# twesterhout/distributed-matvec

Hardware: AMD Instinct MI355X
Metric: matvecs/sec (higher is better)
Workload: dtype f64; 1 GPU; heisenberg_chain_32: y <- H x, 601080390 basis states, 9927521280 off-diagonal non-zeros, f64 vectors, sigma/x/y resident in HBM; partitions=1, partitioning=single, exchange=none, kernel=direct-pull+staged, x=u(hash(sigma, 42)) - 0.5, exchange_bytes_per_matvec=0

## Files before the change

### distributed-matvec_amd/csrc/host.c

```c
#define _GNU_SOURCE
#include <math.h>
#include <pthread.h>
#include <stdarg.h>
#include <stdio.h>
#include <stdlib.h>
#include <string.h>

#include "../../include/ls_amd.h"
#include "../../include/ls_chpl.h"
#include "../../include/ls_hs.h"
#include "lsk.h"

static __thread char g_last_error[1024] = "";
static ls_amd_error_handler g_handler = NULL;

static int set_error(char const *fmt, ...) {
    va_list ap;
    va_start(ap, fmt);
    vsnprintf(g_last_error, sizeof(g_last_error), fmt, ap);
    va_end(ap);
    return -1;
}
static int dev_error(void) { return set_error("%s", lsk_last_error()); }
int ls_amd_internal_error(char const *fmt, ...) {
// ... 1563 lines not shown
    int has_push_staged;
    int one_rank_full_basis;
    lsk_pairplan pairs;
    void *d_pair_recs, *d_rank_low, *d_pair_binom, *d_states32, *d_pair_rows, *d_pair_sites;
    int global_index;
    int has_hubbard;
    lsk_hubbard hubbard;
    void *d_hub[6];
    int has_chain;
    int chain_cached;
    void *d_chain_cache;
    int chain_wide;
    uint64_t *d_chain_rec;
    void *d_chain_wave;
    int chain_row_bytes;
    double chain_v[2];
    int64_t chain_row0;
    void *d_htab;
    uint32_t *d_slot_of;
    int htab_bits;
    void *d_xs;
    int pull_halo;
    int idx_mode;
    struct ls_amd_gtab *gtab;
    uint64_t *d_vtab;
    int64_t row_g0;
    lsk_pullbuf pbuf;
    int64_t split_rows;
    int64_t split_active;
    int slot_cache, slot_cache_valid;
// ... 450 lines not shown
    int64_t slots = 0, total = 0;
    for (int k = 0; k < 8; ++k) if (lists[k].n > slots) slots = lists[k].n;
    uint64_t *flat = (uint64_t *)calloc((size_t)(8 * slots > 0 ? 8 * slots : 1), sizeof(uint64_t));
    for (int k = 0; k < 8; ++k) {
        for (int64_t q = 0; q < lists[k].n; ++q) { flat[k * slots + q] = lists[k].e[q]; total += (int64_t)(lists[k].e[q] >> 48); }
        free(lists[k].e);
    }
    if (total != n) {
        free(flat);
        return set_error("internal error: tile map covers %lld of %lld rows", (long long)total, (long long)n);
    }
    *out = flat;
    *slots_out = slots;
    return 0;
}
static int build_tilemap(ls_amd_plan *pl, int64_t n, int TILE) {
    uint64_t *flat = NULL;
    int64_t slots = 0;
    char const *e = getenv("LS_AMD_TILE_CHUNK");
    int64_t const chunk = e ? atoll(e) : (TILE >= 512 ? 256 : 0);
    if (tilemap_host(n, TILE, chunk > 0 ? chunk : 0, &flat, &slots) < 0) return -1;
    int const up = upload(&pl->d_tilemap, flat, sizeof(uint64_t) * (size_t)(8 * slots > 0 ? 8 * slots : 1));
    free(flat);
    if (up) return -1;
    pl->tilemap.entries = (uint64_t const *)pl->d_tilemap;
    pl->tilemap.slots_per_xcd = slots;
    return 0;
}
int ls_amd_test_corrupt_plan(ls_amd_plan *pl) {
    if (!pl) return 0;
// ... 14 lines not shown
    return 1;
}
int ls_amd_test_window_find(uint64_t const *reps, int n, uint64_t key) { return lsk_test_window_find(reps, n, key); }
int ls_amd_test_nw_find(uint64_t const *reps, int n, uint64_t key) { return lsk_test_nw_find(reps, n, key); }
int ls_amd_test_chain_near_table(int elem, int ldsp, int16_t *out) { return lsk_test_chain_near_table(elem, ldsp, out); }
uint64_t ls_amd_test_rep_trivial_dihedral(uint64_t a, int L, int inv, int reflect) { return lsk_test_rep_trivial_dihedral(a, L, inv, reflect); }
int ls_amd_bench_k4(int L, int inv, int reflect, int variant, int64_t n, uint64_t const *d_reps, uint64_t *d_out, void *stream) {
    if (lsk_bench_k4(L, inv, reflect, variant, n, d_reps, d_out, stream) != 0) { set_error("%s", lsk_last_error()); return -1; }
    return 0;
}
int64_t ls_amd_test_tilemap(int64_t n, int tile_rows, int64_t chunk, uint64_t **entries) {
    int64_t slots = 0;
    *entries = NULL;
    if (tilemap_host(n, tile_rows, chunk, entries, &slots) < 0) return -1;
    return slots;
}
void ls_amd_test_free(void *p) { free(p); }
int ls_amd_test_gtab_bits(int L, int64_t n) { return lsk_gtab_bits(L, n, (int64_t)1 << 40); }
int ls_amd_test_gtab_build(int L, int bbits, int64_t n, uint64_t const *reps, uint32_t const *payload, uint64_t **entries) {
    lsk_gtab t;
    t.entries = NULL; t.L = L; t.bbits = bbits; t.tbits = L - bbits;
    *entries = (uint64_t *)malloc(sizeof(uint64_t) * ((size_t)2 << bbits));
    if (lsk_test_gtab_build_host(t, *entries, n, reps, payload) != 0) { free(*entries); *entries = NULL; return -1; }
    return 0;
}
int64_t ls_amd_test_gtab_find(int L, int bbits, uint64_t const *entries, uint64_t key) {
    lsk_gtab t;
    t.entries = NULL; t.L = L; t.bbits = bbits; t.tbits = L - bbits;
    return lsk_test_gtab_find(t, entries, key);
}
// ... 38 lines not shown
    for (int w = 0; w < 4096; ++w) {
        int const k = __builtin_popcount(w);
        rank_in[w] = (uint16_t)(pos[k] - class_off[k]);
        U[pos[k]++] = (uint16_t)w;
    }
    for (int w = 0; w < 4096; ++w) Rg[w] = low_site >= 0 ? rank_in[w ^ (1 << low_site)] : 0;
}
int ls_amd_test_chain_wave_tables(int low_site, uint16_t *U, uint16_t *Rg, int *class_off) {
    if (low_site >= 12) return set_error("ls_amd_test_chain_wave_tables: the low site lies below bit 12");
    chain_wave_tables(low_site, U, Rg, class_off);
    return 0;
}
static int setup_chain_headers(ls_amd_plan *pl, lsk_index index, int64_t n, uint64_t const *d_reps, int nc, uint64_t xmask, void *stream) {
    int const L = NBITS(pl->op->basis);
    char const *e = getenv("LS_AMD_CHAIN_RECORDS");
    int headed = !(e && atoi(e) != 0) && L >= 13 && L <= 32 && pl->dbs.proj == LSK_PROJ_NONE && pl->chain_row0 == 0 &&
                 pl->family == FAMILY_DIRECT_PULL && pl->dbs.hamming_weight >= 0 && nc <= 1;
    int lo = -1, hi = -1;
    if (headed && nc == 1) {
        lo = __builtin_ctzll(xmask);
        hi = 63 - __builtin_clzll(xmask);
        if (lo >= 12 || hi < 12) { headed = 0; lo = hi = -1; }
    }
    int const words = lsk_chain_words();
    int64_t const n_hdr = (n + 63) / 64;
    uint16_t U[4096], Rg[4096];
    int class_off[14];
    uint32_t *tab = (uint32_t *)malloc(sizeof(uint32_t) * (size_t)words);
    if (!tab) return set_error("out of memory");
    chain_wave_tables(headed ? lo : -1, U, Rg, class_off);
    for (int t = 0; t < words; ++t) tab[t] = (uint32_t)U[t] | ((uint32_t)Rg[U[t]] << 16) | (lo >= 0 ? (((uint32_t)U[t] >> lo) & 1u) << 31 : 0u);
    size_t const tab_bytes = sizeof(uint32_t) * (size_t)words, hdr_bytes = 8 * (size_t)n_hdr;
    void *q;
    if (lsk_malloc(&q, tab_bytes + hdr_bytes + 8) != 0) { free(tab); return 1; }
    unsigned long long plain = 0;
    unsigned long long *d_plain = (unsigned long long *)((char *)q + tab_bytes + hdr_bytes);
    int const rc = lsk_h2d(q, tab, tab_bytes) || lsk_h2d(d_plain, &plain, 8) ||
                   lsk_chain_headers(pl->dbs, index, n, d_reps, headed, hi, (char *)q + tab_bytes, d_plain, stream) || lsk_sync(stream) ||
                   lsk_d2h(&plain, d_plain, 8);
    free(tab);
    if (rc) { lsk_free(q); return dev_error(); }
    pl->d_chain_wave = q;
    int const rec = pl->cplx ? 4 + 4 * nc : 8;
    pl->chain_row_bytes = headed ? (int)((8 * (uint64_t)n_hdr + 64 * (uint64_t)rec * (uint64_t)plain + (uint64_t)n - 1) / (uint64_t)n) : rec;
    return 0;
}
static int setup_chain(ls_amd_plan *pl, lsk_index index, int64_t n, uint64_t const *d_reps, void *stream) {
    struct ls_amd_operator_ext const *ext = OEXT(pl->op);
    int nc = ext->n_groups - ext->runs.n_run_groups;
    int const Ls = NBITS(pl->op->basis);
    int const inv = pl->dbs.proj == LSK_PROJ_INVERSION;
    uint64_t const top = 1ULL << (Ls - 1);
    uint64_t cx[3];
    double cv[3];
    int k = 0;
    if (inv)
        for (int q = 0; q < pl->dop.runs.n_runs; ++q)
            if (pl->dop.runs.lo0[q] + pl->dop.runs.cnt[q] - 1 == Ls - 2) {
                cx[k] = 3ULL << (Ls - 2);
// ... 49 lines not shown
        pl->d_chain_rec = (uint64_t *)q;
        DEV(lsk_chain_pack(n, d_reps, pl->chain_cached ? pl->d_chain_cache : NULL, (uint64_t *)q, stream));
        DEV(lsk_sync(stream));
        if (pl->chain_cached <= 1 && pl->d_chain_cache) { lsk_free(pl->d_chain_cache); pl->d_chain_cache = NULL; }
    }
    if (NBITS(pl->op->basis) <= 32 && !pl->chain_wide && n > 0) {
        int const rc = setup_chain_headers(pl, index, n, d_reps, pl->chain_cached, pl->chain_cached > 0 ? cx[0] : 0, stream);
        if (rc < 0) return -1;
        if (rc > 0) {
            if (pl->d_chain_rec) { lsk_free(pl->d_chain_rec); pl->d_chain_rec = NULL; }
            if (pl->d_chain_cache) { lsk_free(pl->d_chain_cache); pl->d_chain_cache = NULL; }
            if (pl->d_tilemap) { lsk_free(pl->d_tilemap); pl->d_tilemap = NULL; memset(&pl->tilemap, 0, sizeof(pl->tilemap)); }
            pl->chain_cached = 0;
            return 0;
        }
    }
    pl->has_chain = 1;
    return 0;
}

static int pair_cmp(void const *pa, void const *pb) {
    lsk_pair const *a = (lsk_pair const *)pa, *b = (lsk_pair const *)pb;
    int const ca = a->j < 11 ? 0 : (a->i < 11 ? 1 : 2), cb = b->j < 11 ? 0 : (b->i < 11 ? 1 : 2);
    if (ca != cb) return ca - cb;
    if (a->i != b->i) return (int)a->i - (int)b->i;
    return (int)a->j - (int)b->j;
}
static int setup_pairs(ls_amd_plan *pl, int64_t n, uint64_t const *d_reps, void *stream) {
    ls_hs_operator const *op = pl->op;
    struct ls_amd_operator_ext const *ext = OEXT(op);
// ... 815 lines not shown
            if (ps->d_soff) lsk_free(ps->d_soff);
            if (ps->scatter_gt) ls_amd_internal_gtab_release(ps->scatter_gt);
            free(ps->h_soff);
            free(ps->ttab_first);
            free(ps->send_counts); free(ps->h_beta_off); free(ps->h_val_off);
        }
        free(pl->parts);
    }
    if (pl->d_gtable) lsk_free(pl->d_gtable);
    if (pl->d_row_gidx) lsk_free(pl->d_row_gidx);
    if (pl->d_norms_global) lsk_free(pl->d_norms_global);
    if (pl->d_tilemap) lsk_free(pl->d_tilemap);
    if (pl->d_chain_cache) lsk_free(pl->d_chain_cache);
    if (pl->d_chain_rec) lsk_free(pl->d_chain_rec);
    if (pl->d_chain_wave) lsk_free(pl->d_chain_wave);
    if (pl->d_pair_recs) lsk_free(pl->d_pair_recs);
    for (int k = 0; k < 6; ++k) if (pl->d_hub[k]) lsk_free(pl->d_hub[k]);
    if (pl->d_pair_rows) lsk_free(pl->d_pair_rows);
    if (pl->d_pair_sites) lsk_free(pl->d_pair_sites);
    if (pl->d_rank_low) lsk_free(pl->d_rank_low);
    if (pl->d_pair_binom) lsk_free(pl->d_pair_binom);
    if (pl->d_states32) lsk_free(pl->d_states32);
    if (pl->d_htab) lsk_free(pl->d_htab);
    if (pl->d_slot_of) lsk_free(pl->d_slot_of);
    if (pl->d_xs) lsk_free(pl->d_xs);
    if (pl->gtab) ls_amd_internal_gtab_release(pl->gtab);
    split_free(pl);
    block_free(pl);
    if (pl->d_send) lsk_free(pl->d_send);
    if (pl->d_cursors) lsk_free(pl->d_cursors);
// ... 269 lines not shown
    default: return pl->streams ? "tile+streams" : (pl->has_push_staged ? "tile(one rank: push+staged)" : "tile");
    }
}
int ls_amd_plan_packet_bytes(ls_amd_plan const *pl) { return pl->key_bytes + (pl->cplx ? 16 : 8); }
int ls_amd_plan_row_bytes(ls_amd_plan const *pl) {
    if (pl->has_hubbard) return 0;
    if (pl->has_pairs) return pl->pairs.wide ? 8 : 4;
    if (pl->has_chain) {
        if (pl->d_chain_wave) return pl->chain_row_bytes;
        int const narrow = NBITS(pl->op->basis) <= 32 && !pl->chain_wide;
        return (narrow ? 4 : 8) + pl->chain_cached * (pl->chain_wide ? 8 : 4);
    }
    if (pl->family == FAMILY_TILE_PULL || pl->family == FAMILY_REPL_TILE) return 16;
    return 8;
}
int64_t ls_amd_plan_nnz(ls_amd_plan const *pl) { return pl->nnz; }
int ls_amd_plan_send_counts(ls_amd_plan const *pl, int round, int64_t *counts) {
    if (pl->family != FAMILY_TILE) { for (int d = 0; d < pl->P; ++d) counts[d] = 0; return 0; }
    part_state const *ps = &pl->parts[0];
    if (round < 0 || round >= ps->rounds) return set_error("round out of range");
    memcpy(counts, ps->send_counts + (size_t)round * pl->P, sizeof(int64_t) * pl->P);
    return 0;
}

static int prescaled_x(ls_amd_plan *pl, int64_t n, uint64_t const *d_reps, void const *d_x, double const *d_norms,
                       void const **out, void *stream) {
    if (!pl->d_htab) {
        int bits = 4;
        while (((int64_t)1 << bits) < 2 * n) ++bits;
        if (bits > 32) return set_error("hash index: more than 2^31 representatives per table are not supported");
// ... 231 lines not shown
            int const st = stage_begin(pl, ST_DIAG, stream);
            DEV(lsk_memset_async(d_y[0], 0, (size_t)pl->parts[0].count * (pl->cplx ? 16 : 8), stream));
            stage_end(pl, st, stream);
        }
    } else if (pl->family != FAMILY_DIRECT_PULL) {
        int const st = stage_begin(pl, ST_DIAG, stream);
        for (int p = 0; p < pl->n_local; ++p)
            DEV(lsk_diag(pl->dop, pl->cplx, pl->parts[p].count, pl->parts[p].d_reps, d_x[p], d_y[p], stream));
        stage_end(pl, st, stream);
    }
    if (pl->dop.n_groups == 0 && pl->family != FAMILY_DIRECT_PULL) return 0;
    if (pl->family != FAMILY_TILE) {
        part_state *ps = &pl->parts[0];
        int const st = stage_begin(pl, ST_ROWS, stream);
        int slot = timing_begin(pl, stream);
        if (pl->has_chain)
            DEV(lsk_chain(pl->dop, pl->dbs, ps->index, pl->cplx, pl->chain_wide, pl->d_chain_rec != NULL, pl->tilemap, ps->count,
                          pl->d_chain_rec ? pl->d_chain_rec : ps->d_reps, 0, ps->count, d_x[0], d_y[0], pl->chain_cached,
                          pl->d_chain_cache, pl->chain_v[0], pl->chain_v[1], pl->d_chain_wave, stream));
        else if (pl->has_pairs)
            DEV(lsk_pairs(pl->pairs, pl->dbs.hamming_weight, pl->cplx, pl->tilemap, ps->count, d_x[0], d_y[0], stream));
        else if (pl->has_hubbard)
            DEV(lsk_hubbard_apply(pl->hubbard, pl->dop, pl->cplx, pl->tilemap, d_x[0], d_y[0], stream));
        else if (pl->has_push_staged)
            DEV(lsk_push_staged(pl->dop, pl->dbs, ps->index, pl->cplx, pl->tilemap, ps->count, ps->d_reps, d_x[0], d_y[0], pl->d_err, stream));
        else
            DEV(lsk_direct(pl->dop, pl->dbs, ps->index, pl->cplx, pl->family == FAMILY_DIRECT_PULL ? (OEXT(pl->op)->is_hermitian ? 1 : 2) : 0, pl->tilemap, ps->d_reps,
                           d_x[0], d_y[0], pl->d_err, stream));
        timing_end(pl, slot, stream);
        stage_end(pl, st, stream);
        return 0;
    }
    int const P = pl->P;
    if (pl->streams) {
        uint64_t const *d_binom;
// ... 2959 lines not shown
```

### distributed-matvec_amd/csrc/k_rows.hip

```cpp
#include <hip/hip_runtime.h>
#include "lsk_dev.hpp"

template <bool CPLX>
__global__ __launch_bounds__(kBlock) void k_diag(lsk_runs runs, int n_diag, lsk_term const *__restrict__ diag,
                                                 int64_t n, uint64_t const *__restrict__ reps,
                                                 double const *__restrict__ x, double *__restrict__ y) {
    for (int64_t i = (int64_t)blockIdx.x * kBlock + threadIdx.x; i < n; i += (int64_t)gridDim.x * kBlock) {
        uint64_t a = reps[i];
        double dr, di;
        diag_coeff<uint64_t, false>(runs, n_diag, diag, a, dr, di);
        if (CPLX) {
            double xr = x[2 * i], xi = x[2 * i + 1];
            y[2 * i] = dr * xr - di * xi;
            y[2 * i + 1] = dr * xi + di * xr;
        } else {
            y[i] = dr * x[i];
        }
    }
}

extern "C" int lsk_diag(lsk_operator op, int cplx, int64_t n, uint64_t const *reps, void const *x, void *y,
                        void *stream) {
    if (n == 0 || op.n_diag == 0) return 0;
    dim3 g(grid_for(n)), b(kBlock);
// ... 531 lines not shown
}

constexpr int kChainHalo = 512;
constexpr int kChainLdsPairs = 12;
constexpr int kChainFar = 12;
constexpr uint32_t kChainWords = 4096;

__device__ __forceinline__ double cx_load_nt(double const *p) { return __builtin_nontemporal_load(p); }
__device__ __forceinline__ double2 cx_load_nt(double2 const *p) {
    typedef double d2v __attribute__((ext_vector_type(2)));
    const d2v v = __builtin_nontemporal_load(reinterpret_cast<d2v const *>(p));
    return make_double2(v.x, v.y);
}
constexpr int kChainFarC = 6;

template <typename W, typename R, bool CPLX, int TILE, bool REC>
__global__ __launch_bounds__(kBlock, (CPLX || sizeof(R) == 8 ? 5 : (sizeof(W) == 8 ? 6 : 7))) void k_chain_t(lsk_runs runs, int n_diag, lsk_term const *__restrict__ diag,
                                                    int hamming_weight, uint4 const *__restrict__ g_img, int img16, int kc,
                                                    int near_off,
                                                    uint64_t const *__restrict__ tilemap, int64_t slots_per_xcd, int64_t n,
                                                    uint64_t const *__restrict__ reps, void const *__restrict__ x_v,
                                                    void *__restrict__ y_v, int n_cached,
                                                    R const *__restrict__ cache, double cv0, double cv1, int64_t row0,
                                                    int64_t n_x, uint32_t const *__restrict__ wave_plan) {
    typedef typename ChainX<CPLX>::type X;
    typedef WordTraits<W> WT;
    constexpr int NB = ChainTraits<W, R>::NB;
    constexpr int HALO = CPLX ? 256 : kChainHalo;
    constexpr int LDSP = CPLX ? 11 : kChainLdsPairs;
    constexpr int WINDOW = TILE + 2 * HALO + 2;
    constexpr int FAR = CPLX ? kChainFarC : kChainFar;
    constexpr R kNone = ~(R)0;
    constexpr int hb = kChainLdsPairs;
    X const *__restrict__ x = (X const *)x_v;
    X *__restrict__ y = (X *)y_v;
    const bool extra_stream = kAblate && (n_cached & 0x100);
    const int nt_from = !kAblate ? 99 : ((n_cached & 0x200) ? 20 : ((n_cached & 0x400) ? 0 : 99));
    if (kAblate) n_cached &= 0xff;
    uint64_t ex_next = 0;
    extern __shared__ uint4 s_img[];
    R const *const s_binom = reinterpret_cast<R const *>(s_img);
    uint2 const *const s_near = reinterpret_cast<uint2 const *>(reinterpret_cast<char const *>(s_img) + near_off);
    __shared__ X s_x[WINDOW + 1];
    for (int k = threadIdx.x; k < img16; k += kBlock) s_img[k] = g_img[k];
    (void)NB;
    if (threadIdx.x == 0) s_x[WINDOW] = cx_zero<X>();
    const int xcd = blockIdx.x & 7;
    const int64_t blocks_per_xcd = gridDim.x >> 3;
    const int lane = threadIdx.x & 63;
    tilemap += (int64_t)xcd * slots_per_xcd;
    uint32_t const *__restrict__ reps32 = reinterpret_cast<uint32_t const *>(reps);
    constexpr bool HDR = REC || (CPLX && sizeof(W) == 4 && sizeof(R) == 4);
    constexpr int NSUB = TILE / kBlock;
    for (int64_t t = blockIdx.x >> 3; t < slots_per_xcd; t += blocks_per_xcd) {
        const uint64_t slot = tilemap[t];
        const int cnt = (int)(slot >> 48);
        if (cnt == 0) continue;
        const int64_t i0 = (int64_t)(slot & 0xffffffffffffULL);
        const int64_t w0 = (row0 + i0 - HALO) & ~(int64_t)1;
        W a_next = 0;
        R t0_next = kNone, t1_next = kNone;
        auto load_row = [&](int64_t row, W &a_out, R &t0_out, R &t1_out) {
            if (REC) {
                const uint64_t rec = __builtin_nontemporal_load(reps + row);
                a_out = (W)(uint32_t)rec;
                t0_out = (R)(uint32_t)(rec >> 32);
            } else {
                if (sizeof(W) == 4) a_out = (W)__builtin_nontemporal_load(reps32 + 2 * row);
                else a_out = (W)__builtin_nontemporal_load(reps + row);
                if (n_cached > 0) t0_out = __builtin_nontemporal_load(cache + row);
            }
            if (n_cached > 1) t1_out = __builtin_nontemporal_load(cache + (size_t)n + (size_t)row);
            if (kAblate && extra_stream) ex_next = __builtin_nontemporal_load(reps + (row < (n >> 1) ? row + (n >> 1) : row - (n >> 1)));
        };
        const int wave0 = (int)(threadIdx.x & ~63u);
        uint32_t hq = ~0u;
        if (HDR) {
            const uint32_t hw = 2 * (uint32_t)(i0 >> 6) + 2 * ((threadIdx.x >> 6) + (uint32_t)(lane % NSUB) * (kBlock / 64)) + (lane / NSUB) % 2;
            if (((int64_t)(hw >> 1) << 6) < n) hq = wave_plan[kChainWords + hw];
        }
        auto fetch_row = [&](int s, int64_t row) {
            if (HDR) {
                const uint32_t ti = (uint32_t)__builtin_amdgcn_readlane((int)hq, s) & (kChainWords - 1u);
                if (ti != kChainWords - 1u) { a_next = (W)wave_plan[ti + lane]; return; }
            }
            load_row(row, a_next, t0_next, t1_next);
        };
        if (wave0 < cnt) {
            const int64_t rr = i0 + ((int)threadIdx.x < cnt ? (int)threadIdx.x : cnt - 1);
            fetch_row(0, rr);
        }
        __syncthreads();
        if (CPLX) {
            for (int j = threadIdx.x; j < WINDOW; j += kBlock) {
                const int64_t row = w0 + j;
                s_x[j] = (row >= 0 && row < n_x) ? x[row] : cx_zero<X>();
            }
        } else {
            double const *xd = (double const *)x_v;
            double *sd = (double *)s_x;
            for (int j = 2 * threadIdx.x; j < WINDOW; j += 2 * kBlock) {
                const int64_t row = w0 + j;
                double2 v;
                if (row >= 0 && row + 1 < n_x) v = *reinterpret_cast<double2 const *>(xd + row);
                else { v.x = (row >= 0 && row < n_x) ? xd[row] : 0.0; v.y = (row + 1 >= 0 && row + 1 < n_x) ? xd[row + 1] : 0.0; }
                sd[j] = v.x;
                sd[j + 1] = v.y;
            }
        }
        __syncthreads();
        const int own0 = (int)(row0 + i0 - w0);
        X y_pending = cx_zero<X>();
        int r_pending = -1;
#pragma unroll 1
        for (int sub = 0; sub < TILE / kBlock; ++sub) {
            const int r = sub * kBlock + threadIdx.x;
            if (r_pending >= 0) cx_store_nt(y + i0 + r_pending, y_pending);
            r_pending = -1;
            W a = a_next;
            R t0 = t0_next;
            const R t1 = t1_next;
            const uint64_t ex = ex_next;
            if (sub + 1 < TILE / kBlock && (sub + 1) * kBlock + wave0 < cnt) {
                const int64_t in = i0 + (r + kBlock < cnt ? r + kBlock : cnt - 1);
                fetch_row(sub + 1, in);
            }
            if (sub * kBlock + wave0 >= cnt) continue;
            const bool ghost = r >= cnt;
            const int64_t i = i0 + (ghost ? cnt - 1 : r);
            const R ig = (R)(row0 + i);
            W a0;
            int ubit;
            const uint32_t h0 = HDR ? (uint32_t)__builtin_amdgcn_readlane((int)hq, sub) : ~0u;
            if (HDR && (h0 & (kChainWords - 1u)) != kChainWords - 1u) {
                const uint32_t word = (uint32_t)a;
                a0 = (W)(h0 & ~(kChainWords - 1u));
                a = a0 | (W)(word & (kChainWords - 1u));
                ubit = 0;
                const uint32_t h1 = (uint32_t)__builtin_amdgcn_readlane((int)hq, NSUB + sub);
                t0 = (int32_t)(word ^ h1) < 0 ? (R)((h1 & 0x7fffffffu) + ((word >> 16) & 0x7fffu)) : kNone;
            } else {
                a0 = readfirstlane_t<W>(a);
                const W adiff = a0 ^ readlane_t<W>(a, 63);
                ubit = adiff == 0 ? 0 : (int)(8 * sizeof(W)) - (sizeof(W) == 4 ? __clz((int)(uint32_t)adiff) : __clzll((long long)(uint64_t)adiff));
            }
            const int jr = own0 + (int)(i - i0);
            const X xr = s_x[jr];
            X g0 = n_cached > 0 ? xr : cx_zero<X>(), g1 = n_cached > 1 ? xr : cx_zero<X>();
            if (t0 != kNone) g0 = x[t0];
            if (n_cached > 1 && t1 != kNone) g1 = x[t1];
            double dr, di;
            diag_coeff<W, true>(runs, n_diag, diag, a, dr, di);
            X acc = cx_scale(dr, xr);
            const W tdiff = a ^ (a >> 1);
            const R ig0 = readfirstlane_t<R>(ig);
            const uint32_t dl = (uint32_t)(ig - ig0);
            for (int q = 0; q < runs.n_runs; ++q) {
                const int lo0 = runs.lo0[q];
                int lo_end = lo0 + runs.cnt[q];
                const double vr = runs.v_re[q];
                int k = WT::popc(a & (W)(((uint64_t)1 << lo0) - 1));
                int lo = lo0;
                const int e1 = lo_end < LDSP ? lo_end : LDSP;
                const int near_end = lo0 > e1 ? lo0 : e1;
                int split = hb == 0 ? lo_end : (hb < near_end ? near_end : (hb > lo_end ? lo_end : hb));
                if (hb != 0 && split < ubit) split = ubit < lo_end ? ubit : lo_end;
                const bool uni = split < lo_end;
                unsigned long long m = 0;
                R off = 0;
                X xv[FAR];
#pragma unroll
                for (int u = 0; u < FAR; ++u) xv[u] = cx_zero<X>();
                if (uni) {
                    const int p = split + lane;
                    const bool in_run = p < lo_end;
                    const int ps = in_run ? p : 0;
                    const W hi = a0 >> ps;
                    const bool bit = hi & 1;
                    const bool act = in_run && (((hi >> 1) & 1) != (W)bit);
                    const int kk = hamming_weight - WT::popc(hi);
                    const R d = s_binom[ps * kc + (kk < 0 ? 0 : kk)];
                    off = bit ? d : (R)(0 - d);
                    m = __builtin_amdgcn_ballot_w64(act);
#pragma unroll
                    for (int u = 0; u < FAR; ++u) {
                        if (m) {
                            const int l = __builtin_ctzll(m);
                            m &= m - 1;
                            X const *const src = x + (size_t)(R)(ig0 + readlane_t<R>(off, l)) + dl;
                            if (kAblate && split + l >= nt_from) xv[u] = cx_load_nt(src); else xv[u] = *src;
                        }
                    }
                    lo_end = split;
                }
// ... 23 lines not shown
                        for (int u = 0; u < NBATCH; ++u)
                            if (p0 + u < LDSP) cx_fma(vr, nv[u], acc);
                    }
                    lo = LDSP;
                    k = __popc(al & ((1u << LDSP) - 1u));
                }
#pragma unroll 4
                for (; lo < e1; ++lo) {
                    const bool bit = (a >> lo) & 1;
                    const bool act = (tdiff >> lo) & 1;
                    const int d = (int)s_binom[lo * kc + k];
                    k += bit ? 1 : 0;
                    const int j = bit ? jr + d : jr - d;
                    cx_fma(vr, s_x[act ? j : WINDOW], acc);
                }
#pragma unroll
                for (int u = 0; u < FAR; ++u) cx_fma(vr, xv[u], acc);
                while (m) {
                    X xw[4];
#pragma unroll
                    for (int u = 0; u < 4; ++u) {
                        xw[u] = cx_zero<X>();
                        if (m) {
                            const int l = __builtin_ctzll(m);
                            m &= m - 1;
                            xw[u] = (x + (size_t)(R)(ig0 + readlane_t<R>(off, l)))[dl];
                        }
                    }
#pragma unroll
                    for (int u = 0; u < 4; ++u) cx_fma(vr, xw[u], acc);
                }
#pragma unroll 4
                for (; lo < lo_end; ++lo) {
                    const bool bit = (a >> lo) & 1;
                    const bool act = (tdiff >> lo) & 1;
                    const R d = s_binom[lo * kc + k];
                    k += bit ? 1 : 0;
                    R idx = bit ? (R)(ig + d) : (R)(ig - d);
                    idx = act ? idx : ig;
                    cx_fma(act ? vr : 0.0, x[idx], acc);
                }
            }
            cx_fma(t0 != kNone ? cv0 : 0.0, g0, acc);
            cx_fma(t1 != kNone ? cv1 : 0.0, g1, acc);
            if (kAblate && extra_stream && ex == 0x0123456789abcdefULL) cx_fma(1.0, xr, acc);
            y_pending = acc;
            r_pending = ghost ? -1 : r;
        }
        if (r_pending >= 0) cx_store_nt(y + i0 + r_pending, y_pending);
    }
}

template <typename W, typename R>
__global__ __launch_bounds__(kBlock) void k_chain_cache(int64_t n, uint64_t const *__restrict__ reps, uint64_t xmask, uint64_t inv_mask,
                                                        int hamming_weight, uint64_t const *__restrict__ g_binom,
                                                        R *__restrict__ out, int *__restrict__ flag) {
    constexpr int NB = ChainTraits<W, R>::NB;
    __shared__ R s_binom[NB * LSK_BINOM_K];
    for (int k = threadIdx.x; k < NB * LSK_BINOM_K; k += blockDim.x) s_binom[k] = (R)g_binom[k];
    __syncthreads();
    for (int64_t i = (int64_t)blockIdx.x * kBlock + threadIdx.x; i < n; i += (int64_t)gridDim.x * kBlock) {
        const W a = (W)reps[i];
        R t = ~(R)0;
        if (WordTraits<W>::popc(a & (W)xmask) == 1) {
            W beta = a ^ (W)xmask;
// ... 176 lines not shown
    if (n == 0 || tm.slots_per_xcd == 0) return 0;
    const bool narrow = bs.number_sites <= 32 && !wide_ranks;
    if ((wave_plan != nullptr) != narrow) { snprintf(g_err, sizeof(g_err), "lsk_chain: 32-bit states and ranks come with wave headers, the other plans without"); return -1; }
#define LSK_CHAIN_ARGS op, bs, ix, tm, n, reps, row0, n_x, x, y, n_cached, cache, cv0, cv1, wave_plan, stream
    if (fused_records) {
        if (!narrow || cplx) { snprintf(g_err, sizeof(g_err), "lsk_chain: fused records need 32-bit states and ranks and f64 vectors"); return -1; }
        return launch_chain<uint32_t, uint32_t, false, 1024, true>(LSK_CHAIN_ARGS);
    }
    if (narrow) {
        if (!cplx) { snprintf(g_err, sizeof(g_err), "lsk_chain: 32-bit states and ranks with f64 vectors run on fused records (lsk_chain_pack)"); return -1; }
        return launch_chain<uint32_t, uint32_t, true, 512, false>(LSK_CHAIN_ARGS);
    }
    if (!wide_ranks) return cplx ? launch_chain<uint64_t, uint32_t, true, 512, false>(LSK_CHAIN_ARGS) : launch_chain<uint64_t, uint32_t, false, 1024, false>(LSK_CHAIN_ARGS);
    return cplx ? launch_chain<uint64_t, uint64_t, true, 512, false>(LSK_CHAIN_ARGS) : launch_chain<uint64_t, uint64_t, false, 1024, false>(LSK_CHAIN_ARGS);
#undef LSK_CHAIN_ARGS
}

constexpr int kPairLowBits = 11;
constexpr int kPairHalo = 512;
constexpr int kPairFar = 8;
enum { PAIR_NEAR = 0, PAIR_STRADDLE = 1, PAIR_HIGH = 2 };

template <typename SW, bool CPLX, int TILE>
__global__ __launch_bounds__(kBlock, (CPLX ? 4 : 6)) void k_pairs_t(lsk_pairplan pp, int hamming_weight, uint64_t const *__restrict__ tilemap,
                                                              int64_t slots_per_xcd, int64_t n, void const *__restrict__ x_v,
                                                              void *__restrict__ y_v) {
    typedef typename ChainX<CPLX>::type X;
    constexpr int HALO = kPairHalo;
    constexpr int WINDOW = TILE + 2 * HALO + 2;
    constexpr int LOWMASK = (1 << kPairLowBits) - 1;
// ... 452 lines not shown
```

### distributed-matvec_amd/csrc/lsk.h

```cpp
#ifndef LSK_H
#define LSK_H

#include <stddef.h>
#include <stdint.h>

#ifdef __cplusplus
extern "C" {
#endif

#define LSK_BENES_STAGES 11
#define LSK_BINOM_K 34
#define LSK_MAX_PARTS 256

typedef struct lsk_term {
    double v_re, v_im;
    uint64_t m, r, s;
} lsk_term;

enum { LSK_GROUP_GENERIC = 0, LSK_GROUP_EXCHANGE = 1,
       LSK_GROUP_HOP_LO = 2, LSK_GROUP_HOP_HI = 3 };

typedef struct lsk_group {
    uint64_t x;
    double v_re, v_im;
// ... 150 lines not shown
int lsk_event_destroy(void *ev);
int lsk_event_record(void *ev, void *stream);
int lsk_event_elapsed_ms(void *start, void *stop, float *ms);

int lsk_fill_random(int64_t n, uint64_t const *states, uint64_t seed, int cplx, void *out, void *stream);

int lsk_diag(lsk_operator op, int cplx, int64_t n, uint64_t const *reps, void const *x, void *y,
             void *stream);
int lsk_direct_validate(lsk_operator op, lsk_basis bs, lsk_index ix, int64_t n, uint64_t const *reps, int *d_err, void *stream);
int lsk_direct(lsk_operator op, lsk_basis bs, lsk_index ix, int cplx, int pull, lsk_tilemap tm,
               uint64_t const *reps, void const *x, void *y, int *d_err, void *stream);
int lsk_chain_tile_rows(int cplx);
int lsk_chain(lsk_operator op, lsk_basis bs, lsk_index ix, int cplx, int wide_ranks, int fused_records, lsk_tilemap tm,
              int64_t n, uint64_t const *reps, int64_t row0, int64_t n_x, void const *x, void *y, int n_cached,
              void const *cache, double cv0, double cv1, void const *wave_plan, void *stream);
#define LSK_MAX_PAIRS 128
#define LSK_PAIR_KC 20
typedef struct lsk_pair {
    uint8_t i, j, pad[6];
    double v;
    double vz;
} lsk_pair;
typedef struct lsk_pair_row {
    uint64_t between;
    double v, vz;
    int i, j;
} lsk_pair_row;
#define LSK_PAIR_SITE_MAX_DEGREE 8
#define LSK_PAIR_SITE_MAX_CLASSES 64
typedef struct lsk_pairplan {
// ... 375 lines not shown
```

### include/ls_amd.h

```cpp
#ifndef LS_AMD_H
#define LS_AMD_H

#include "ls_hs.h"

#ifdef __cplusplus
extern "C" {
#endif

typedef enum { LS_AMD_F64 = 0, LS_AMD_C128 = 1 } ls_amd_dtype;

typedef enum {
    LS_AMD_MODE_AUTO = 0,
    LS_AMD_MODE_PUSH = 1,
    LS_AMD_MODE_PULL = 2
} ls_amd_mode;

typedef struct ls_amd_plan ls_amd_plan;

char const *ls_amd_last_error(void);
typedef void (*ls_amd_error_handler)(char const *message);
void ls_amd_set_error_handler(ls_amd_error_handler handler);

int ls_amd_device_count(void);
int ls_amd_set_device(int device);
// ... 245 lines not shown
int ls_amd_expect_matrix_elements(ls_amd_expect *plan, ls_amd_dtype dtype, int Ka, void const *d_bra, int64_t bra_row, int64_t bra_col,
                                  int Kb, void const *d_ket, int64_t ket_row, int64_t ket_col, double *h_out, void *stream);
char const *ls_amd_expect_matrix_kernel_name(ls_amd_expect const *plan, int Ka, int Kb);
int64_t ls_amd_test_expect_average(ls_hs_basis const *basis, ls_hs_operator const *op, int64_t cap, double *v, uint64_t *m, uint64_t *r,
                                   uint64_t *x, uint64_t *s);

int ls_amd_basis_group_order(ls_hs_basis const *basis);
int ls_amd_basis_fermion_signs(ls_hs_basis const *basis);
int ls_amd_test_fermion_sign(ls_hs_basis const *basis, int element, uint64_t state, int table);
int ls_amd_basis_spin_flip(ls_hs_basis const *basis);
int ls_amd_test_group_element_kind(ls_hs_basis const *basis, int element);
uint64_t ls_amd_basis_apply_group_element(ls_hs_basis const *basis, int element, uint64_t state);
int ls_amd_basis_group_character(ls_hs_basis const *basis, int element, double *re, double *im);

int64_t ls_amd_test_tilemap(int64_t n, int tile_rows, int64_t chunk, uint64_t **entries);
void ls_amd_test_free(void *p);
int ls_amd_test_window_find(uint64_t const *reps, int n, uint64_t key);
int ls_amd_test_nw_find(uint64_t const *reps, int n, uint64_t key);
int ls_amd_test_chain_near_table(int elem, int ldsp, int16_t *out);
int ls_amd_test_chain_wave_tables(int low_site, uint16_t *U, uint16_t *Rg, int *class_off);
uint64_t ls_amd_test_rep_trivial_dihedral(uint64_t a, int L, int inv, int reflect);
int ls_amd_bench_k4(int L, int inv, int reflect, int variant, int64_t n, uint64_t const *d_reps, uint64_t *d_out, void *stream);
int ls_amd_test_translation_cosets(ls_hs_basis const *basis, int *n_cosets);
uint64_t ls_amd_test_rep_by_cosets(ls_hs_basis const *basis, uint64_t state);
int ls_amd_test_d4_mask(ls_hs_basis const *basis);
int ls_amd_test_gtab_bits(int L, int64_t n);
int ls_amd_test_gtab_build(int L, int bbits, int64_t n, uint64_t const *reps, uint32_t const *payload, uint64_t **entries);
int64_t ls_amd_test_gtab_find(int L, int bbits, uint64_t const *entries, uint64_t key);
int ls_amd_test_primme_comminfo_offset(void);
int ls_amd_test_primme_sumtype_offset(void);
// ... 8 lines not shown
```

Baseline: 142.2 matvecs/s.

## Pair chain tiles across the top-bond offset so far hops stay in LDS

For the Heisenberg chain, rows in a middle index range whose top-bond (site L-2) hop lands a fixed distance d away are processed in paired tiles. Each tile loads two x windows into LDS, one at i0 and one at i0+d, so the top-bond partner and most bit-LDSP hops are read from shared memory instead of through gathered global loads. A separate tile map covers the remaining rows, and a second kernel launch with its own header array handles the paired rows. The cost is more setup, a larger LDS window per block, and an extra launch. Correctness now depends on the binomial ordering of the basis.

```diff
diff --git a/distributed-matvec_amd/csrc/host.c b/distributed-matvec_amd/csrc/host.c
--- a/distributed-matvec_amd/csrc/host.c
+++ b/distributed-matvec_amd/csrc/host.c
@@ -1601,6 +1601,12 @@
     uint64_t *d_chain_rec;
     void *d_chain_wave;
     int chain_row_bytes;
+    int chain_headed;
+    int chain_headers_apply;
+    int chain_paired;
+    void *d_tilemap_pair, *d_chain_hdr_b;
+    lsk_tilemap tilemap_pair;
+    int64_t chain_pair_d, chain_pair_a0, chain_pair_rows;
     double chain_v[2];
     int64_t chain_row0;
     void *d_htab;
@@ -2081,6 +2087,64 @@
     *slots_out = slots;
     return 0;
 }
+static int chain_pair_range(int L, int k, int64_t *a0, int64_t *a1, int64_t *d) {
+    if (L < 14 || L > 32 || k < 1 || k > L - 1) return 0;
+    uint64_t C[33][33];
+    memset(C, 0, sizeof(C));
+    for (int n = 0; n <= 32; ++n) { C[n][0] = 1; for (int j = 1; j <= n; ++j) C[n][j] = C[n - 1][j - 1] + (j <= n - 1 ? C[n - 1][j] : 0); }
+    int64_t const r01 = (int64_t)C[L - 2][k], r10 = (int64_t)C[L - 1][k];
+    *d = r10 - r01;
+    *a0 = (r01 + 511) & ~(int64_t)511;
+    *a1 = r10 & ~(int64_t)511;
+    return *a1 > *a0;
+}
+#define CHAIN_TILE_PLAIN 0x8000
+static int tilemap_deal(tile_list const *all, int64_t chunk, uint64_t **out, int64_t *slots_out) {
+    int64_t const tiles = all->n;
+    int64_t per[8] = {0, 0, 0, 0, 0, 0, 0, 0}, slots = 0;
+    if (chunk > 0) for (int64_t q = 0; q < tiles; ++q) ++per[(q / chunk) % 8];
+    else for (int k = 0; k < 8; ++k) per[k] = tiles * (k + 1) / 8 - tiles * k / 8;
+    for (int k = 0; k < 8; ++k) if (per[k] > slots) slots = per[k];
+    uint64_t *flat = (uint64_t *)calloc((size_t)(8 * slots > 0 ? 8 * slots : 1), sizeof(uint64_t));
+    if (!flat) return set_error("out of memory");
+    int64_t fill[8] = {0, 0, 0, 0, 0, 0, 0, 0};
+    int k0 = 0;
+    for (int64_t q = 0; q < tiles; ++q) {
+        int k;
+        if (chunk > 0) k = (int)((q / chunk) % 8);
+        else { while (q >= tiles * (k0 + 1) / 8) ++k0; k = k0; }
+        flat[k * slots + fill[k]++] = all->e[q];
+    }
+    *out = flat;
+    *slots_out = slots;
+    return 0;
+}
+static int tilemap_paired_host(int64_t n, int TILE, int64_t chunk, int64_t a0, int64_t a1, int64_t d, uint64_t **rest, int64_t *rest_slots,
+                               uint64_t **pairs, int64_t *pair_slots) {
+    tile_list all[2];
+    memset(all, 0, sizeof(all));
+    int64_t const piece[3][2] = {{0, a0}, {a1, a0 + d}, {a1 + d, n}};
+    int64_t total = 0;
+    for (int p = 0; p < 3; ++p)
+        for (int64_t pos = piece[p][0]; pos < piece[p][1];) {
+            int64_t end = (pos / TILE + 1) * TILE;
+            if (pos & 63) end = (pos | 63) + 1;
+            if (end > piece[p][1]) end = piece[p][1];
+            int const plain = (pos & 63) != 0 || ((end & 63) != 0 && end != n);
+            tile_push(&all[0], pos, (end - pos) | (plain ? CHAIN_TILE_PLAIN : 0));
+            total += end - pos;
+            pos = end;
+        }
+    for (int64_t i0 = a0; i0 < a1; i0 += 512) { tile_push(&all[1], i0, 1024); total += 1024; }
+    int rc = total == n ? 0 : set_error("internal error: paired tile maps cover %lld of %lld rows", (long long)total, (long long)n);
+    *rest = *pairs = NULL;
+    if (!rc) rc = tilemap_deal(&all[0], chunk, rest, rest_slots);
+    if (!rc) rc = tilemap_deal(&all[1], chunk, pairs, pair_slots);
+    if (rc) { free(*rest); free(*pairs); *rest = *pairs = NULL; }
+    free(all[0].e);
+    free(all[1].e);
+    return rc;
+}
 static int build_tilemap(ls_amd_plan *pl, int64_t n, int TILE) {
     uint64_t *flat = NULL;
     int64_t slots = 0;
@@ -2125,6 +2189,15 @@
     *entries = NULL;
     if (tilemap_host(n, tile_rows, chunk, entries, &slots) < 0) return -1;
     return slots;
+}
+int ls_amd_test_tilemap_paired(int L, int weight, int tile_rows, int64_t chunk, uint64_t **rest, uint64_t **pairs, int64_t *out) {
+    int64_t a0, a1, d, n = 1;
+    *rest = *pairs = NULL;
+    if (!chain_pair_range(L, weight, &a0, &a1, &d)) return 0;
+    for (int j = 1; j <= weight; ++j) n = n * (L - weight + j) / j;
+    if (tilemap_paired_host(n, tile_rows, chunk, a0, a1, d, rest, &out[4], pairs, &out[5]) != 0) return -1;
+    out[0] = n; out[1] = a0; out[2] = a1; out[3] = d;
+    return 1;
 }
 void ls_amd_test_free(void *p) { free(p); }
 int ls_amd_test_gtab_bits(int L, int64_t n) { return lsk_gtab_bits(L, n, (int64_t)1 << 40); }
@@ -2193,7 +2266,7 @@
 static int setup_chain_headers(ls_amd_plan *pl, lsk_index index, int64_t n, uint64_t const *d_reps, int nc, uint64_t xmask, void *stream) {
     int const L = NBITS(pl->op->basis);
     char const *e = getenv("LS_AMD_CHAIN_RECORDS");
-    int headed = !(e && atoi(e) != 0) && L >= 13 && L <= 32 && pl->dbs.proj == LSK_PROJ_NONE && pl->chain_row0 == 0 &&
+    int headed = L >= 13 && L <= 32 && pl->dbs.proj == LSK_PROJ_NONE && pl->chain_row0 == 0 &&
                  pl->family == FAMILY_DIRECT_PULL && pl->dbs.hamming_weight >= 0 && nc <= 1;
     int lo = -1, hi = -1;
     if (headed && nc == 1) {
@@ -2201,6 +2274,8 @@
         hi = 63 - __builtin_clzll(xmask);
         if (lo >= 12 || hi < 12) { headed = 0; lo = hi = -1; }
     }
+    pl->chain_headers_apply = headed;
+    if (e && atoi(e) != 0) { headed = 0; lo = hi = -1; }
     int const words = lsk_chain_words();
     int64_t const n_hdr = (n + 63) / 64;
     uint16_t U[4096], Rg[4096];
@@ -2220,8 +2295,59 @@
     free(tab);
     if (rc) { lsk_free(q); return dev_error(); }
     pl->d_chain_wave = q;
+    pl->chain_headed = headed;
     int const rec = pl->cplx ? 4 + 4 * nc : 8;
     pl->chain_row_bytes = headed ? (int)((8 * (uint64_t)n_hdr + 64 * (uint64_t)rec * (uint64_t)plain + (uint64_t)n - 1) / (uint64_t)n) : rec;
+    return 0;
+}
+static int setup_chain_pairs(ls_amd_plan *pl, lsk_index index, int64_t n, uint64_t const *d_reps, int hi, void *stream) {
+    char const *e = getenv("LS_AMD_CHAIN_PAIRED");
+    int const L = NBITS(pl->op->basis);
+    if ((e && atoi(e) == 0) || !pl->chain_headers_apply || pl->cplx || !pl->d_chain_rec || pl->chain_cached > 1 || pl->chain_row0 != 0 ||
+        pl->n_local != 1 || pl->family != FAMILY_DIRECT_PULL)
+        return 0;
+    int top = 0;
+    for (int q = 0; q < pl->dop.runs.n_runs; ++q)
+        if (pl->dop.runs.lo0[q] <= L - 2 && L - 2 < pl->dop.runs.lo0[q] + pl->dop.runs.cnt[q]) top = 1;
+    int64_t a0, a1, d;
+    if (!top || !chain_pair_range(L, pl->dbs.hamming_weight, &a0, &a1, &d) || a1 + d > n) return 0;
+    uint64_t *rest = NULL, *pairs = NULL;
+    int64_t rest_slots = 0, pair_slots = 0;
+    char const *ce = getenv("LS_AMD_TILE_CHUNK");
+    int64_t const chunk = ce ? atoll(ce) : 256;
+    if (tilemap_paired_host(n, lsk_chain_tile_rows(0), chunk > 0 ? chunk : 0, a0, a1, d, &rest, &rest_slots, &pairs, &pair_slots) != 0) return -1;
+    void *d_rest = NULL, *d_pairs = NULL, *d_hdr = NULL;
+    int64_t const n_b = a1 - a0;
+    unsigned long long plain = 0;
+    int rc = lsk_malloc(&d_rest, sizeof(uint64_t) * (size_t)(8 * rest_slots > 0 ? 8 * rest_slots : 1)) ||
+             lsk_malloc(&d_pairs, sizeof(uint64_t) * (size_t)(8 * pair_slots)) || lsk_malloc(&d_hdr, 8 * (size_t)(n_b / 64) + 8);
+    if (!rc) {
+        unsigned long long *d_plain = (unsigned long long *)((char *)d_hdr + 8 * (size_t)(n_b / 64));
+        rc = lsk_h2d(d_rest, rest, sizeof(uint64_t) * (size_t)(8 * rest_slots)) || lsk_h2d(d_pairs, pairs, sizeof(uint64_t) * (size_t)(8 * pair_slots)) ||
+             lsk_h2d(d_plain, &plain, 8) || lsk_chain_headers(pl->dbs, index, n_b, d_reps + a0 + d, pl->chain_headed, hi, d_hdr, d_plain, stream) ||
+             lsk_sync(stream);
+        if (rc) { free(rest); free(pairs); lsk_free(d_rest); lsk_free(d_pairs); lsk_free(d_hdr); return dev_error(); }
+    }
+    free(rest);
+    free(pairs);
+    if (rc) {
+        if (d_rest) lsk_free(d_rest);
+        if (d_pairs) lsk_free(d_pairs);
+        if (d_hdr) lsk_free(d_hdr);
+        return 0;
+    }
+    lsk_free(pl->d_tilemap);
+    pl->d_tilemap = d_rest;
+    pl->tilemap.entries = (uint64_t const *)d_rest;
+    pl->tilemap.slots_per_xcd = rest_slots;
+    pl->d_tilemap_pair = d_pairs;
+    pl->tilemap_pair.entries = (uint64_t const *)d_pairs;
+    pl->tilemap_pair.slots_per_xcd = pair_slots;
+    pl->d_chain_hdr_b = d_hdr;
+    pl->chain_pair_d = d;
+    pl->chain_pair_a0 = a0;
+    pl->chain_pair_rows = 2 * (a1 - a0);
+    pl->chain_paired = 1;
     return 0;
 }
 static int setup_chain(ls_amd_plan *pl, lsk_index index, int64_t n, uint64_t const *d_reps, void *stream) {
@@ -2301,6 +2427,7 @@
             pl->chain_cached = 0;
             return 0;
         }
+        if (setup_chain_pairs(pl, index, n, d_reps, pl->chain_cached > 0 ? 63 - __builtin_clzll(cx[0]) : -1, stream) != 0) return -1;
     }
     pl->has_chain = 1;
     return 0;
@@ -3146,6 +3273,8 @@
     if (pl->d_chain_cache) lsk_free(pl->d_chain_cache);
     if (pl->d_chain_rec) lsk_free(pl->d_chain_rec);
     if (pl->d_chain_wave) lsk_free(pl->d_chain_wave);
+    if (pl->d_tilemap_pair) lsk_free(pl->d_tilemap_pair);
+    if (pl->d_chain_hdr_b) lsk_free(pl->d_chain_hdr_b);
     if (pl->d_pair_recs) lsk_free(pl->d_pair_recs);
     for (int k = 0; k < 6; ++k) if (pl->d_hub[k]) lsk_free(pl->d_hub[k]);
     if (pl->d_pair_rows) lsk_free(pl->d_pair_rows);
@@ -3445,6 +3574,9 @@
     if (pl->family == FAMILY_TILE_PULL || pl->family == FAMILY_REPL_TILE) return 16;
     return 8;
 }
+int64_t ls_amd_plan_chain_paired_rows(ls_amd_plan const *pl) {
+    return pl->has_chain && pl->chain_paired ? pl->chain_pair_rows : 0;
+}
 int64_t ls_amd_plan_nnz(ls_amd_plan const *pl) { return pl->nnz; }
 int ls_amd_plan_send_counts(ls_amd_plan const *pl, int round, int64_t *counts) {
     if (pl->family != FAMILY_TILE) { for (int d = 0; d < pl->P; ++d) counts[d] = 0; return 0; }
@@ -3706,11 +3838,14 @@
         part_state *ps = &pl->parts[0];
         int const st = stage_begin(pl, ST_ROWS, stream);
         int slot = timing_begin(pl, stream);
-        if (pl->has_chain)
+        if (pl->has_chain) {
             DEV(lsk_chain(pl->dop, pl->dbs, ps->index, pl->cplx, pl->chain_wide, pl->d_chain_rec != NULL, pl->tilemap, ps->count,
                           pl->d_chain_rec ? pl->d_chain_rec : ps->d_reps, 0, ps->count, d_x[0], d_y[0], pl->chain_cached,
                           pl->d_chain_cache, pl->chain_v[0], pl->chain_v[1], pl->d_chain_wave, stream));
-        else if (pl->has_pairs)
+            if (pl->chain_paired)
+                DEV(lsk_chain_paired(pl->dop, pl->dbs, pl->tilemap_pair, ps->count, pl->d_chain_rec, d_x[0], d_y[0], pl->chain_cached, pl->chain_v[0],
+                                     pl->d_chain_wave, pl->chain_pair_d, pl->chain_pair_a0, pl->d_chain_hdr_b, NBITS(pl->op->basis) - 2, stream));
+        } else if (pl->has_pairs)
             DEV(lsk_pairs(pl->pairs, pl->dbs.hamming_weight, pl->cplx, pl->tilemap, ps->count, d_x[0], d_y[0], stream));
         else if (pl->has_hubbard)
             DEV(lsk_hubbard_apply(pl->hubbard, pl->dop, pl->cplx, pl->tilemap, d_x[0], d_y[0], stream));
diff --git a/distributed-matvec_amd/csrc/k_rows.hip b/distributed-matvec_amd/csrc/k_rows.hip
--- a/distributed-matvec_amd/csrc/k_rows.hip
+++ b/distributed-matvec_amd/csrc/k_rows.hip
@@ -569,21 +569,25 @@
 }
 constexpr int kChainFarC = 6;
 
-template <typename W, typename R, bool CPLX, int TILE, bool REC>
-__global__ __launch_bounds__(kBlock, (CPLX || sizeof(R) == 8 ? 5 : (sizeof(W) == 8 ? 6 : 7))) void k_chain_t(lsk_runs runs, int n_diag, lsk_term const *__restrict__ diag,
+struct chain_pair_args { int64_t d, a0; uint32_t const *hdr_b; int bond; };
+template <typename W, typename R, bool CPLX, int TILE, bool REC, bool PAIR>
+__device__ __forceinline__ void chain_rows(lsk_runs const &runs, int n_diag, lsk_term const *__restrict__ diag,
                                                     int hamming_weight, uint4 const *__restrict__ g_img, int img16, int kc,
                                                     int near_off,
                                                     uint64_t const *__restrict__ tilemap, int64_t slots_per_xcd, int64_t n,
                                                     uint64_t const *__restrict__ reps, void const *__restrict__ x_v,
                                                     void *__restrict__ y_v, int n_cached,
                                                     R const *__restrict__ cache, double cv0, double cv1, int64_t row0,
-                                                    int64_t n_x, uint32_t const *__restrict__ wave_plan) {
+                                                    int64_t n_x, uint32_t const *__restrict__ wave_plan, chain_pair_args const &pr) {
     typedef typename ChainX<CPLX>::type X;
     typedef WordTraits<W> WT;
     constexpr int NB = ChainTraits<W, R>::NB;
-    constexpr int HALO = CPLX ? 256 : kChainHalo;
-    constexpr int LDSP = CPLX ? 11 : kChainLdsPairs;
-    constexpr int WINDOW = TILE + 2 * HALO + 2;
+    constexpr int HALO = (CPLX || PAIR) ? 256 : kChainHalo;
+    constexpr int LDSP = (CPLX || PAIR) ? 11 : kChainLdsPairs;
+    constexpr int SEG = TILE / 2;
+    constexpr int WSEG = SEG + 2 * HALO + 2;
+    constexpr int WINDOW = PAIR ? 2 * WSEG : TILE + 2 * HALO + 2;
+    static_assert(!PAIR || (REC && !CPLX && SEG % kBlock == 0 && SEG % 64 == 0), "paired tiles: f64 on fused records");
     constexpr int FAR = CPLX ? kChainFarC : kChainFar;
     constexpr R kNone = ~(R)0;
     constexpr int hb = kChainLdsPairs;
@@ -609,10 +613,13 @@
     constexpr int NSUB = TILE / kBlock;
     for (int64_t t = blockIdx.x >> 3; t < slots_per_xcd; t += blocks_per_xcd) {
         const uint64_t slot = tilemap[t];
-        const int cnt = (int)(slot >> 48);
-        if (cnt == 0) continue;
+        const int cnt_slot = REC ? (int)((slot >> 48) & 0x7ffu) : (int)(slot >> 48);
+        if (cnt_slot == 0) continue;
+        const int cnt = PAIR ? TILE : cnt_slot;
         const int64_t i0 = (int64_t)(slot & 0xffffffffffffULL);
         const int64_t w0 = (row0 + i0 - HALO) & ~(int64_t)1;
+        const int64_t w0b = PAIR ? (i0 + pr.d - HALO) & ~(int64_t)1 : 0;
+        auto row_off = [&](int s) -> int { return PAIR ? (s >> 1) * (int)pr.d + (s & 1) * kBlock + (int)threadIdx.x : s * kBlock + threadIdx.x; };
         W a_next = 0;
         R t0_next = kNone, t1_next = kNone;
         auto load_row = [&](int64_t row, W &a_out, R &t0_out, R &t1_out) {
@@ -630,7 +637,12 @@
         };
         const int wave0 = (int)(threadIdx.x & ~63u);
         uint32_t hq = ~0u;
-        if (HDR) {
+        if (PAIR) {
+            const uint32_t s = (uint32_t)lane % NSUB;
+            const uint32_t wr = (threadIdx.x >> 6) + (s & 1u) * (kBlock / 64);
+            const uint32_t word = ((uint32_t)lane / NSUB) % 2;
+            hq = (s >> 1) ? pr.hdr_b[2 * ((uint32_t)((i0 - pr.a0) >> 6) + wr) + word] : wave_plan[kChainWords + 2 * ((uint32_t)(i0 >> 6) + wr) + word];
+        } else if (HDR && !(REC && (slot >> 63))) {
             const uint32_t hw = 2 * (uint32_t)(i0 >> 6) + 2 * ((threadIdx.x >> 6) + (uint32_t)(lane % NSUB) * (kBlock / 64)) + (lane / NSUB) % 2;
             if (((int64_t)(hw >> 1) << 6) < n) hq = wave_plan[kChainWords + hw];
         }
@@ -655,7 +667,7 @@
             double const *xd = (double const *)x_v;
             double *sd = (double *)s_x;
             for (int j = 2 * threadIdx.x; j < WINDOW; j += 2 * kBlock) {
-                const int64_t row = w0 + j;
+                const int64_t row = (PAIR && j >= WSEG) ? w0b + (j - WSEG) : w0 + j;
                 double2 v;
                 if (row >= 0 && row + 1 < n_x) v = *reinterpret_cast<double2 const *>(xd + row);
                 else { v.x = (row >= 0 && row < n_x) ? xd[row] : 0.0; v.y = (row + 1 >= 0 && row + 1 < n_x) ? xd[row + 1] : 0.0; }
@@ -665,23 +677,26 @@
         }
         __syncthreads();
         const int own0 = (int)(row0 + i0 - w0);
+        const int own0b = PAIR ? WSEG + (int)(i0 + pr.d - w0b) : 0;
         X y_pending = cx_zero<X>();
         int r_pending = -1;
 #pragma unroll 1
         for (int sub = 0; sub < TILE / kBlock; ++sub) {
-            const int r = sub * kBlock + threadIdx.x;
+            const int r = row_off(sub);
             if (r_pending >= 0) cx_store_nt(y + i0 + r_pending, y_pending);
             r_pending = -1;
             W a = a_next;
             R t0 = t0_next;
             const R t1 = t1_next;
             const uint64_t ex = ex_next;
-            if (sub + 1 < TILE / kBlock && (sub + 1) * kBlock + wave0 < cnt) {
+            if (PAIR) {
+                if (sub + 1 < TILE / kBlock) fetch_row(sub + 1, i0 + row_off(sub + 1));
+            } else if (sub + 1 < TILE / kBlock && (sub + 1) * kBlock + wave0 < cnt) {
                 const int64_t in = i0 + (r + kBlock < cnt ? r + kBlock : cnt - 1);
                 fetch_row(sub + 1, in);
             }
-            if (sub * kBlock + wave0 >= cnt) continue;
-            const bool ghost = r >= cnt;
+            if (!PAIR && sub * kBlock + wave0 >= cnt) continue;
+            const bool ghost = !PAIR && r >= cnt;
             const int64_t i = i0 + (ghost ? cnt - 1 : r);
             const R ig = (R)(row0 + i);
             W a0;
@@ -699,7 +714,9 @@
                 const W adiff = a0 ^ readlane_t<W>(a, 63);
                 ubit = adiff == 0 ? 0 : (int)(8 * sizeof(W)) - (sizeof(W) == 4 ? __clz((int)(uint32_t)adiff) : __clzll((long long)(uint64_t)adiff));
             }
-            const int jr = own0 + (int)(i - i0);
+            const int jl = PAIR ? (sub & 1) * kBlock + (int)threadIdx.x : 0;
+            const int jr = PAIR ? ((sub >> 1) ? own0b : own0) + jl : own0 + (int)(i - i0);
+            const int jp = PAIR ? ((sub >> 1) ? own0 : own0b) + jl : 0;
             const X xr = s_x[jr];
             X g0 = n_cached > 0 ? xr : cx_zero<X>(), g1 = n_cached > 1 ? xr : cx_zero<X>();
             if (t0 != kNone) g0 = x[t0];
@@ -714,6 +731,7 @@
                 const int lo0 = runs.lo0[q];
                 int lo_end = lo0 + runs.cnt[q];
                 const double vr = runs.v_re[q];
+                const bool top_here = PAIR && lo0 <= pr.bond && pr.bond < lo_end;
                 int k = WT::popc(a & (W)(((uint64_t)1 << lo0) - 1));
                 int lo = lo0;
                 const int e1 = lo_end < LDSP ? lo_end : LDSP;
@@ -732,7 +750,7 @@
                     const int ps = in_run ? p : 0;
                     const W hi = a0 >> ps;
                     const bool bit = hi & 1;
-                    const bool act = in_run && (((hi >> 1) & 1) != (W)bit);
+                    const bool act = in_run && (((hi >> 1) & 1) != (W)bit) && !(PAIR && p == pr.bond);
                     const int kk = hamming_weight - WT::popc(hi);
                     const R d = s_binom[ps * kc + (kk < 0 ? 0 : kk)];
                     off = bit ? d : (R)(0 - d);
@@ -786,6 +804,21 @@
                     const int j = bit ? jr + d : jr - d;
                     cx_fma(vr, s_x[act ? j : WINDOW], acc);
                 }
+                if (PAIR && lo == LDSP && lo < lo_end) {
+                    const bool bit = (a >> LDSP) & 1;
+                    const bool act = (tdiff >> LDSP) & 1;
+                    const int d = (int)s_binom[LDSP * kc + k];
+                    const int j = bit ? jr + d : jr - d;
+                    const int sb = (sub >> 1) * WSEG;
+                    if (__builtin_amdgcn_ballot_w64(act && (j < sb || j >= sb + WSEG)) == 0)
+                        cx_fma(vr, s_x[act ? j : WINDOW], acc);
+                    else {
+                        const R idx = act ? (bit ? (R)(ig + (R)d) : (R)(ig - (R)d)) : ig;
+                        cx_fma(act ? vr : 0.0, x[idx], acc);
+                    }
+                    k += bit ? 1 : 0;
+                    ++lo;
+                }
 #pragma unroll
                 for (int u = 0; u < FAR; ++u) cx_fma(vr, xv[u], acc);
                 while (m) {
@@ -802,6 +835,7 @@
 #pragma unroll
                     for (int u = 0; u < 4; ++u) cx_fma(vr, xw[u], acc);
                 }
+                if (top_here) cx_fma(vr, s_x[jp], acc);
 #pragma unroll 4
                 for (; lo < lo_end; ++lo) {
                     const bool bit = (a >> lo) & 1;
@@ -821,6 +855,27 @@
         }
         if (r_pending >= 0) cx_store_nt(y + i0 + r_pending, y_pending);
     }
+}
+template <typename W, typename R, bool CPLX, int TILE, bool REC>
+__global__ __launch_bounds__(kBlock, (CPLX || sizeof(R) == 8 ? 5 : (sizeof(W) == 8 ? 6 : 7))) void k_chain_t(lsk_runs runs, int n_diag, lsk_term const *__restrict__ diag,
+                                                    int hamming_weight, uint4 const *__restrict__ g_img, int img16, int kc,
+                                                    int near_off,
+                                                    uint64_t const *__restrict__ tilemap, int64_t slots_per_xcd, int64_t n,
+                                                    uint64_t const *__restrict__ reps, void const *__restrict__ x_v,
+                                                    void *__restrict__ y_v, int n_cached,
+                                                    R const *__restrict__ cache, double cv0, double cv1, int64_t row0,
+                                                    int64_t n_x, uint32_t const *__restrict__ wave_plan) {
+    chain_rows<W, R, CPLX, TILE, REC, false>(runs, n_diag, diag, hamming_weight, g_img, img16, kc, near_off, tilemap, slots_per_xcd, n, reps, x_v, y_v,
+                                             n_cached, cache, cv0, cv1, row0, n_x, wave_plan, chain_pair_args{0, 0, nullptr, -1});
+}
+__global__ __launch_bounds__(kBlock, 7) void k_chain_pair_t(lsk_runs runs, int n_diag, lsk_term const *__restrict__ diag, int hamming_weight,
+                                                            uint4 const *__restrict__ g_img, int img16, int kc, int near_off,
+                                                            uint64_t const *__restrict__ tilemap, int64_t slots_per_xcd, int64_t n,
+                                                            uint64_t const *__restrict__ reps, void const *__restrict__ x_v,
+                                                            void *__restrict__ y_v, int n_cached, double cv0, chain_pair_args pr,
+                                                            uint32_t const *__restrict__ wave_plan) {
+    chain_rows<uint32_t, uint32_t, false, 1024, true, true>(runs, n_diag, diag, hamming_weight, g_img, img16, kc, near_off, tilemap, slots_per_xcd, n,
+                                                            reps, x_v, y_v, n_cached, nullptr, cv0, 0.0, 0, n, wave_plan, pr);
 }
 
 template <typename W, typename R>
@@ -1027,6 +1082,23 @@
     if (!wide_ranks) return cplx ? launch_chain<uint64_t, uint32_t, true, 512, false>(LSK_CHAIN_ARGS) : launch_chain<uint64_t, uint32_t, false, 1024, false>(LSK_CHAIN_ARGS);
     return cplx ? launch_chain<uint64_t, uint64_t, true, 512, false>(LSK_CHAIN_ARGS) : launch_chain<uint64_t, uint64_t, false, 1024, false>(LSK_CHAIN_ARGS);
 #undef LSK_CHAIN_ARGS
+}
+extern "C" int lsk_chain_paired(lsk_operator op, lsk_basis bs, lsk_tilemap tm_pair, int64_t n, uint64_t const *records, void const *x, void *y,
+                                int n_cached, double cv0, void const *wave_plan, int64_t d, int64_t a0, void const *hdr_b, int bond, void *stream) {
+    if (n == 0 || tm_pair.slots_per_xcd == 0) return 0;
+    if (bs.number_sites < 14 || bs.number_sites > 32 || bond != bs.number_sites - 2 || n_cached > 1 || !wave_plan || !hdr_b || !tm_pair.entries ||
+        d < 512 || (a0 & 511) || a0 + d + 512 > n) {
+        snprintf(g_err, sizeof(g_err), "lsk_chain_paired: plan out of range");
+        return -1;
+    }
+    ChainImage img;
+    if (chain_lds_image(4, ChainTraits<uint32_t, uint32_t>::NB, bs.hamming_weight, 8, 11, &img) != 0) return -1;
+    chain_pair_args pr = {d, a0, (uint32_t const *)hdr_b, bond};
+    hipLaunchKernelGGL(k_chain_pair_t, dim3((unsigned)(tm_pair.slots_per_xcd * 8)), dim3(kBlock), (size_t)img.bytes, (hipStream_t)stream, op.runs,
+                       op.n_diag, op.diag, bs.hamming_weight, img.dev, img.bytes / 16, img.kc, img.near_off, tm_pair.entries,
+                       tm_pair.slots_per_xcd, n, records, x, y, n_cached, cv0, pr, (uint32_t const *)wave_plan);
+    LSK_LAUNCH_CHECK();
+    return 0;
 }
 
 constexpr int kPairLowBits = 11;
diff --git a/distributed-matvec_amd/csrc/lsk.h b/distributed-matvec_amd/csrc/lsk.h
--- a/distributed-matvec_amd/csrc/lsk.h
+++ b/distributed-matvec_amd/csrc/lsk.h
@@ -188,6 +188,8 @@
 int lsk_chain(lsk_operator op, lsk_basis bs, lsk_index ix, int cplx, int wide_ranks, int fused_records, lsk_tilemap tm,
               int64_t n, uint64_t const *reps, int64_t row0, int64_t n_x, void const *x, void *y, int n_cached,
               void const *cache, double cv0, double cv1, void const *wave_plan, void *stream);
+int lsk_chain_paired(lsk_operator op, lsk_basis bs, lsk_tilemap tm_pair, int64_t n, uint64_t const *records, void const *x, void *y,
+                     int n_cached, double cv0, void const *wave_plan, int64_t d, int64_t a0, void const *hdr_b, int bond, void *stream);
 #define LSK_MAX_PAIRS 128
 #define LSK_PAIR_KC 20
 typedef struct lsk_pair {
diff --git a/include/ls_amd.h b/include/ls_amd.h
--- a/include/ls_amd.h
+++ b/include/ls_amd.h
@@ -283,6 +283,8 @@
 int ls_amd_basis_group_character(ls_hs_basis const *basis, int element, double *re, double *im);
 
 int64_t ls_amd_test_tilemap(int64_t n, int tile_rows, int64_t chunk, uint64_t **entries);
+int64_t ls_amd_plan_chain_paired_rows(ls_amd_plan const *pl);
+int ls_amd_test_tilemap_paired(int L, int weight, int tile_rows, int64_t chunk, uint64_t **rest, uint64_t **pairs, int64_t *out);
 void ls_amd_test_free(void *p);
 int ls_amd_test_window_find(uint64_t const *reps, int n, uint64_t key);
 int ls_amd_test_nw_find(uint64_t const *reps, int n, uint64_t key);
```

New measurement: 144.7 matvecs/s (median of 6 runs). +1.8%, better.
